# MiloszKrajewski/K4os.Compression.LZ4

Measured on AMD Instinct MI355X. Metric: GiB/s encode+decode on batched 64 KiB blocks; bit-exact vs C# ref, higher is better.
Workload: dtype u8

## Files before the change

### k4os/compression/lz4_amd/csrc/k4lz4_capi.hip

```cpp
#include <hip/hip_runtime.h>
#include <stdint.h>
#include <stdio.h>
#include <stdlib.h>
#include <string.h>
#include <algorithm>
#include <atomic>
#include <memory>
#include <new>
#include <condition_variable>
#include <functional>
#include <mutex>
#include <string>
#include <thread>
#include <chrono>
#include <vector>

#include "../../../../include/k4lz4.h"
#include "k4lz4_decode.hpp"
#include "k4lz4_encode_fast.hpp"
#include "k4lz4_parse.hpp"
#include "k4lz4_pickle.hpp"
#include "k4lz4_segments.hpp"
#include "k4lz4_encode_hc.hpp"
#include "k4lz4_fast_chain.hpp"
// ... 10 lines not shown
#include "k4lz4_selftest.hpp"

constexpr int MAX_PARTS = 8;

struct k4lz4_ctx {
    int device = -1;
    std::string error;
    hipStream_t stream = nullptr;
    int accel = 1;
    unsigned long long *prof = nullptr;
    bool prof_pair = false;
    bool prof_stamp = false;
    uint8_t *d_src = nullptr; size_t d_src_cap = 0;
    uint8_t *d_dst = nullptr; size_t d_dst_cap = 0;
    uint8_t *d_meta = nullptr; size_t d_meta_cap = 0;
    uint8_t *h_stage = nullptr; size_t h_stage_cap = 0;
    uint8_t *d_sched = nullptr; size_t d_sched_cap = 0;
    int cu_count = 256;
    uint8_t *d_dict = nullptr; size_t d_dict_cap = 0;
    uint8_t *d_gtab = nullptr; size_t d_gtab_cap = 0;
    hipStream_t aux = nullptr;
    hipStream_t aux2 = nullptr;
    hipEvent_t ev_join2 = nullptr;
    uint8_t *d_seg = nullptr; size_t d_seg_cap = 0;
    uint8_t *d_seg_first = nullptr; size_t d_seg_first_cap = 0;
    bool use_segments = true;
    uint32_t seg_min = 1024u << 10, seg_target = 640u << 10, seg_warm = 384u << 10;
    uint32_t seg_target_max = 1408u << 10;
    uint32_t seg_spin_max = 0;
    uint32_t seg_div = 3500;
    hipEvent_t ev_fork = nullptr, ev_join = nullptr;
    uint8_t *d_hc_hash = nullptr; size_t d_hc_hash_cap = 0;
    uint8_t *d_hc_work = nullptr; size_t d_hc_work_cap = 0;
    uint8_t *d_hc_meta = nullptr; size_t d_hc_meta_cap = 0;
    uint8_t *d_pk_meta = nullptr; size_t d_pk_meta_cap = 0;
    int pickle_split_min = 512;
    hipEvent_t ev_busy = nullptr;
    hipStream_t last_stream = nullptr;
    bool busy = false;
    uint64_t hc_res_total = 0; uint32_t hc_res_longest = 0;
    uint8_t *h_in[2] = {nullptr, nullptr}; size_t h_in_cap[2] = {0, 0};
    uint8_t *h_out[2] = {nullptr, nullptr}; size_t h_out_cap[2] = {0, 0};
    hipEvent_t ev_in[2] = {nullptr, nullptr}, ev_out[2] = {nullptr, nullptr};
    uint8_t *d_pack = nullptr; size_t d_pack_cap = 0;
    hipStream_t copyq = nullptr;
    hipStream_t dlq = nullptr;
    hipEvent_t ev_up[MAX_PARTS] = {}, ev_len[MAX_PARTS] = {};
    uint8_t *h_len = nullptr; size_t h_len_cap = 0;
    struct Pool *pool = nullptr, *pool_dl = nullptr;
    bool pool_failed = false, pool_dl_failed = false;
    int stage_threads = 7;
    uint32_t *d_pace = nullptr;
    uint32_t *d_status = nullptr;
    int split_pct = -1;
    bool no_pair = false;
    int direct_span_pct = 200;
    bool no_direct = false;
    int lds_floor_per_cu = 8;
    int cost_pct = 48;
    int dec_parts = 4, dec_parts_direct = 8;
    int hop2_max_per_cu = 12;
    bool hc_cand_lds = true;
    int hc_cand_dynlds = 0;
    int hc_segs = 0;
    bool hc_chain_parts = true;
    int hc_mem_pct = 33;
    int pace_min_per_cu = 6;
    bool use_pace = true;
    bool prof_gtab = false;
    uint8_t *d_parse = nullptr; size_t d_parse_cap = 0;
    bool use_parse = true;
    bool parse_queue = false;
    bool hc_records = true;
    bool parse_seg = true;
    bool parse_big = true;
    bool parse_persist = true;
    bool parse_inline_emit = true;
    bool parse_migrate = true;
    bool parse_pcost = false;
    int parse_waves = 16;
    bool trace = false;
    std::vector<uint8_t> h_chain;
    uint8_t *d_chain = nullptr; size_t d_chain_cap = 0;
    hipEvent_t ev_chain = nullptr;
    uint8_t *d_fr = nullptr; size_t d_fr_cap = 0;
    uint8_t *d_fb = nullptr; size_t d_fb_cap = 0;
    uint8_t *d_lg = nullptr; size_t d_lg_cap = 0;
    uint8_t *d_frd = nullptr; size_t d_frd_cap = 0;
    uint8_t *d_lgr = nullptr; size_t d_lgr_cap = 0;
    uint8_t *d_lga = nullptr; size_t d_lga_cap = 0;
    std::vector<uint8_t> h_fw;
    uint8_t *d_fw = nullptr; size_t d_fw_cap = 0;
    hipEvent_t ev_fw = nullptr;
};

struct Pool {
    std::vector<std::thread> workers;
    std::mutex m;
    std::condition_variable cv_work, cv_done;
    std::function<void(int)> job;
    int parts = 0, next = 0, pending = 0;
    unsigned long long gen = 0;
    bool stop = false;
    explicit Pool(int nthreads)
    {
        for (int t = 0; t < nthreads; t++) workers.emplace_back([this] { run(); });
    }
    ~Pool()
    {
        { std::lock_guard<std::mutex> g(m); stop = true; }
        cv_work.notify_all();
        for (auto &w : workers) w.join();
    }
    void run()
    {
        std::unique_lock<std::mutex> lk(m);
        for (;;) {
            cv_work.wait(lk, [this] { return stop || next < parts; });
            if (stop) return;
            const int i = next++;
            lk.unlock();
            job(i);
            lk.lock();
            if (--pending == 0) cv_done.notify_all();
        }
    }
    void parallel(int nparts, const std::function<void(int)> &f)
    {
        if (nparts <= 1 || workers.empty()) { for (int i = 0; i < nparts; i++) f(i); return; }
        std::unique_lock<std::mutex> lk(m);
// ... 344 lines not shown
        if (((kind == KIND_ENCODE && !parse_path) || (K4_DEC_PACE && (kind == KIND_DECODE || kind == KIND_UNPICKLE))) && ctx->use_pace && ctx->d_pace && cnt > (int64_t)ctx->pace_min_per_cu * (int64_t)ctx->cu_count) {
            a.pace = ctx->d_pace;
            K4_HIP(ctx, hipMemsetAsync(a.pace, 0, k4::PACE_BYTES, stream));
        }
        k4::SegArgs sg{};
        bool seg = false;
        if (kind == KIND_ENCODE && (flags & (FLAG_SEGMENTS_OK | K4LZ4_FLAG_SEGMENTS)) && ctx->use_segments && !a.prof && !(flags & K4LZ4_FLAG_ALLOW_COPY)) {
            static_assert(k4::SEG_HDR_DWORDS * 4 == 256, "seg_first_of finds the header in front of the items");
            size_t max_items = (size_t)k4::SEG_MAX_ITEMS;
            if (hostLen) {
                size_t bound = 0;
                for (int64_t i = 0; i < cnt && bound < max_items; i++) {
                    const int32_t u = hostLen[first + i];
                    if (u > 0 && (uint32_t)u >= ctx->seg_min) bound += ((size_t)u + ctx->seg_target - 1) / ctx->seg_target;
                }
                max_items = std::min(max_items, std::max<size_t>(bound, 2));
            }
            const size_t o_items = 256, o_work = o_items + max_items * sizeof(k4::SegItem);
            const size_t o_blocks = o_work + max_items * 4, o_snaps = (o_blocks + (size_t)k4::SEG_MAX_BLOCKS * 4 + 255) & ~(size_t)255;
            const size_t o_tables = o_snaps + max_items * k4::SEG_SNAP_DWORDS * 4, total = o_tables + max_items * 16384;
            if (total > ctx->d_seg_cap || (size_t)cnt * 4 > ctx->d_seg_first_cap) {
                K4_HIP(ctx, hipStreamSynchronize(stream));
                K4_HIP(ctx, hipStreamSynchronize(ctx->aux2));
            }
            int rc = grow(ctx, &ctx->d_seg, &ctx->d_seg_cap, total, false);
            if (rc == K4LZ4_OK) rc = grow(ctx, &ctx->d_seg_first, &ctx->d_seg_first_cap, (size_t)cnt * 4, false);
            if (rc != K4LZ4_OK) return rc;
            sg.hdr = (k4::SegHdr *)ctx->d_seg; sg.items = (k4::SegItem *)(ctx->d_seg + o_items); sg.work = (uint32_t *)(ctx->d_seg + o_work);
            sg.blocks = (uint32_t *)(ctx->d_seg + o_blocks); sg.snaps = (uint32_t *)(ctx->d_seg + o_snaps); sg.tables = (uint32_t *)(ctx->d_seg + o_tables);
            sg.first = (int32_t *)ctx->d_seg_first;
            sg.seg_min = ctx->seg_min; sg.seg_target = ctx->seg_target; sg.seg_warm = ctx->seg_warm; sg.seg_div = ctx->seg_div; sg.seg_target_max = ctx->seg_target_max; sg.spin_max = ctx->seg_spin_max; sg.max_items = (uint32_t)max_items;
            hipLaunchKernelGGL(k4::k4_seg_plan_kernel, dim3(1), dim3(256), 0, stream, a, sg);
            a.seg_first = sg.first; a.seg_items = sg.items; a.seg_snaps = sg.snaps;
            seg = true;
        }
        auto segments_start = [&]() -> int {
            if (!seg) return K4LZ4_OK;
            K4_HIP(ctx, hipEventRecord(ctx->ev_fork, stream));
            K4_HIP(ctx, hipStreamWaitEvent(ctx->aux2, ctx->ev_fork, 0));
            hipLaunchKernelGGL(k4::k4_encode_seg_kernel, dim3((unsigned)((sg.max_items + k4::ENCODE_WAVES_PER_WG - 1) / k4::ENCODE_WAVES_PER_WG)), dim3(64 * k4::ENCODE_WAVES_PER_WG), 0, ctx->aux2, a, sg);
            K4_HIP(ctx, hipEventRecord(ctx->ev_join2, ctx->aux2));
            return K4LZ4_OK;
        };
        auto segments_join = [&]() -> int {
            if (!seg) return K4LZ4_OK;
            K4_HIP(ctx, hipStreamWaitEvent(stream, ctx->ev_join2, 0));
            hipLaunchKernelGGL(k4::k4_seg_join_kernel, dim3((unsigned)std::min<int64_t>(k4::SEG_MAX_BLOCKS, cnt)), dim3(64), 0, stream, a, sg);
            return K4LZ4_OK;
        };
        if (dd && dd->dict) {
            a.dict = dd->dict; a.dictOff = dd->off + first; a.dictLen = dd->len + first;
            a.dictMode = dd->mode ? dd->mode + first : nullptr;
        }
        if (reorder && parse_path && kind == KIND_ENCODE && ctx->parse_pcost) {
            a.cost = d_cost; a.hist = d_hist; a.order_out = d_order;
            K4_HIP(ctx, hipMemsetAsync(d_hist, 0, 2 * k4::PCOST_BUCKETS * 4, stream));
            hipLaunchKernelGGL(k4::k4_pcost_kernel, dim3((unsigned)((cnt + k4::PCOST_WAVES_PER_WG - 1) / k4::PCOST_WAVES_PER_WG)), dim3(64 * k4::PCOST_WAVES_PER_WG), 0, stream, a);
            hipLaunchKernelGGL(k4::k4_porder_kernel, dim3((unsigned)((cnt + 255) / 256)), dim3(256), 0, stream, a);
            a.order = d_order;
        }
        else if (reorder) {
            a.cost = d_cost; a.hist = d_hist; a.order_out = d_order;
            K4_HIP(ctx, hipMemsetAsync(d_hist, 0, (2 * k4::COST_BUCKETS + 16) * 4, stream));
            hipLaunchKernelGGL(k4::k4_cost_kernel, dim3((unsigned)cnt), dim3(64), 0, stream, a, encode_like ? 0 : 1,
                               kind == KIND_ENCODE && parse_path ? k4::COST_SAMPLE_PARSE : k4::COST_SAMPLE);
            const bool two_kernels = kind == KIND_ENCODE && !a.prof && cnt > 512 && !(flags & K4LZ4_FLAG_NO_SPLIT) &&
                                     cnt > 8 * (int64_t)ctx->cu_count && ctx->split_pct <= 0;
            k4::BatchArgs ao = a;
            ao.first = two_kernels ? (uint32_t)ctx->cost_pct : 0u;
            ao.total = (uint32_t)((int64_t)ctx->lds_floor_per_cu * (int64_t)ctx->cu_count);
            hipLaunchKernelGGL(k4::k4_order_kernel, dim3((unsigned)((cnt + 255) / 256)), dim3(256), 0, stream, ao, (uint32_t)lds_share(ctx, cnt));
            a.order = d_order;
            if (two_kernels) a.split = d_hist + 2 * k4::COST_BUCKETS;
        }
        const unsigned wg4 = (unsigned)((cnt + k4::DECODE_WAVES_PER_WG - 1) / k4::DECODE_WAVES_PER_WG);
        bool parse_here = kind == KIND_ENCODE && (parse_path || (parse_seg_path && (a.order || cnt == 1)));
        const bool big_ok = ctx->parse_big && ctx->parse_inline_emit;
        bool any_small = true, any_big = big_ok;
        if (parse_here && hostLen) {
            any_small = false; any_big = false;
            for (int64_t i = 0; i < cnt && !(any_small && (any_big || !big_ok)); i++) {
                const int32_t len = hostLen[first + i];
                if (len >= (int32_t)k4::PARSE_MIN_LEN && len < k4::LIMIT_64K) any_small = true;
                else if (len >= k4::LIMIT_64K && big_ok) any_big = true;
            }
            parse_here = any_small || any_big;
        }
        int64_t waves = 0, nwg = 0, nwg_seg = 0;
        const bool seg_two_step = seg && parse_here && parse_seg_path;
        bool queue = false, slot_recs = false;
        size_t o_meta = 0, o_gtab = 0;
        if (parse_here) {
            waves = std::max<int64_t>(1, std::min<int64_t>(ctx->parse_waves, (cnt + ctx->cu_count - 1) / ctx->cu_count));
            queue = (ctx->parse_queue || parse_persistent || parse_seg_path) && a.order && cnt > waves * (int64_t)ctx->cu_count;
            nwg = queue ? (int64_t)ctx->cu_count : (cnt + waves - 1) / waves;
            if (seg_two_step) nwg_seg = std::min<int64_t>(ctx->cu_count, (cnt + (int64_t)sg.max_items + k4::PARSE_MAX_WAVES - 1) / k4::PARSE_MAX_WAVES);
            slot_recs = ctx->parse_inline_emit;
            const size_t rec_slots = slot_recs ? std::max((size_t)nwg * (size_t)waves, (size_t)nwg_seg * k4::PARSE_MAX_WAVES) : (size_t)cnt;
            o_meta = rec_slots * k4::PARSE_REC_STRIDE * sizeof(uint2); o_gtab = (o_meta + (size_t)cnt * 8 + 64 + 255) & ~(size_t)255;
            const size_t need = o_gtab + std::max(waves > k4::PARSE_LDS_TABLES ? (size_t)nwg * k4::PARSE_MAX_WAVES * 16384 : 0, (size_t)nwg_seg * k4::PARSE_MAX_WAVES * 16384);
            if (need > ctx->d_parse_cap) K4_HIP(ctx, hipStreamSynchronize(stream));
            const int rcp = grow(ctx, &ctx->d_parse, &ctx->d_parse_cap, need, false);
            if (rcp != K4LZ4_OK) { std::lock_guard<std::mutex> g(g_err_mu); ctx->error.clear(); parse_here = false; }
        }
        if (parse_here) {
            k4::ParseArgs pa{};
            pa.recs = (uint2 *)ctx->d_parse; pa.meta = (uint32_t *)(ctx->d_parse + o_meta); pa.gtab = (uint32_t *)(ctx->d_parse + o_gtab);
            pa.nwg = (uint32_t)nwg;
            pa.inline_emit = ctx->parse_inline_emit ? 1u : 0u;
            pa.slot_recs = slot_recs ? 1u : 0u;
            pa.migrate = ctx->parse_migrate ? 1u : 0u;
            pa.big = any_big ? 1u : 0u;
            K4_HIP(ctx, hipMemsetAsync(pa.meta + 2 * cnt, 0, 32, stream));
            if (queue) pa.queue = pa.meta + 2 * cnt;
            pa.nbig = pa.meta + 2 * cnt + 3;
            hipLaunchKernelGGL(k4::k4_parse_kernel, dim3((unsigned)nwg), dim3((unsigned)(64 * waves)), 0, stream, a, pa);
            if (seg_two_step) {
                k4::ParseArgs pb = pa;
                pb.queue = pa.meta + 2 * cnt + 4;
                pb.nwg = (uint32_t)nwg_seg;
                hipLaunchKernelGGL(k4::k4_parse_seg_kernel, dim3((unsigned)nwg_seg), dim3(64 * k4::PARSE_MAX_WAVES), 0, stream, a, pb, sg);
            } else if (any_big) {
                k4::ParseArgs pb = pa;
                if (queue) pb.queue = pa.queue + 4;
                hipLaunchKernelGGL(k4::k4_parse_big_kernel, dim3((unsigned)nwg), dim3((unsigned)(64 * waves)), 0, stream, a, pb);
            }
            if (!pa.inline_emit)
                hipLaunchKernelGGL(k4::k4_emit_kernel, dim3((unsigned)((cnt + k4::EMIT_WAVES_PER_WG - 1) / k4::EMIT_WAVES_PER_WG)), dim3(64 * k4::EMIT_WAVES_PER_WG), 0, stream, a, pa);
            bool rest = true;
            if (hostLen) {
                rest = false;
                for (int64_t i = 0; i < cnt && !rest; i++) rest = hostLen[first + i] < (int32_t)k4::PARSE_MIN_LEN || (hostLen[first + i] >= k4::LIMIT_64K && !any_big);
            }
            if (rest)
                hipLaunchKernelGGL(k4::k4_encode_fast_rest_kernel, dim3((unsigned)((cnt + k4::ENCODE_WAVES_PER_WG - 1) / k4::ENCODE_WAVES_PER_WG)), dim3(64 * k4::ENCODE_WAVES_PER_WG), 0, stream, a, pa);
            if (seg_two_step)
                hipLaunchKernelGGL(k4::k4_seg_join_kernel, dim3((unsigned)std::min<int64_t>(k4::SEG_MAX_BLOCKS, cnt)), dim3(64), 0, stream, a, sg);
            if (flags & K4LZ4_FLAG_ALLOW_COPY)
                hipLaunchKernelGGL(k4::k4_allow_copy_kernel, dim3((unsigned)((cnt + 3) / 4)), dim3(256), 0, stream, a);
            K4_HIP(ctx, hipGetLastError());
            continue;
        }
        switch (kind) {
        case KIND_ENCODE:
            if (a.prof && !ctx->prof_stamp) {
                if (ctx->prof_gtab) {
                    if ((size_t)cnt * 16384 > ctx->d_gtab_cap) {
                        K4_HIP(ctx, hipStreamSynchronize(ctx->aux));
                        int rc2 = grow(ctx, &ctx->d_gtab, &ctx->d_gtab_cap, (size_t)cnt * 16384, false);
                        if (rc2 != K4LZ4_OK) return rc2;
                    }
                    a.gtab = (uint32_t *)ctx->d_gtab;
                }
                hipLaunchKernelGGL(k4::k4_encode_fast_prof_kernel, dim3((unsigned)cnt), dim3(64), 0, stream, a);
            }
            else if (reorder && cnt > 512 && !(flags & K4LZ4_FLAG_NO_SPLIT)) {
                const int64_t lds_slots = 8 * (int64_t)ctx->cu_count;
                const int64_t n_lds = lds_share(ctx, cnt);
                const int64_t n_g = cnt - (a.split ? std::min<int64_t>(cnt, (int64_t)ctx->lds_floor_per_cu * (int64_t)ctx->cu_count) : n_lds);
                const int64_t gchunk = 8192;
                if (n_g > 0 && (size_t)std::min(n_g, gchunk) * 16384 > ctx->d_gtab_cap) {
                    K4_HIP(ctx, hipStreamSynchronize(ctx->aux));
                    int rc2 = grow(ctx, &ctx->d_gtab, &ctx->d_gtab_cap, (size_t)std::min(n_g, gchunk) * 16384, false);
                    if (rc2 != K4LZ4_OK) return rc2;
                }
                { const int rcs = segments_start(); if (rcs != K4LZ4_OK) return rcs; }
// ... 1046 lines not shown
        return rc;
    return s.finish({{outLen, d_out, (size_t)n * 8}}, dst, dstOff, [&](int64_t i) {
        return outLen[i] > 0 && (!capped || (uint64_t)outLen[i] <= dstCap[i]) ? (size_t)outLen[i] : 0;
    });
}

using k4::FW_XXH_BYTES; using k4::FW_CHAIN_LIMIT; using k4::FwAfter;
using k4::fw_ring_at; using k4::fw_slot; using k4::fw_header; using k4::fw_opens; using k4::fw_model; using k4::fw_bound; using k4::fw_code;
using k4::fw_advance;

size_t fw_take(size_t &at, size_t bytes) { const size_t o = at; at += (bytes + 255) & ~(size_t)255; return o; }

}

extern "C" {

int k4lz4_version(void) { return K4LZ4_VERSION; }

void k4lz4_set_enforce32(int on) { g_enforce32.store(on ? 1 : 0, std::memory_order_relaxed); }
int k4lz4_get_enforce32(void) { return g_enforce32.load(std::memory_order_relaxed); }

int k4lz4_device_count(void)
{
    int n = 0;
    if (hipGetDeviceCount(&n) != hipSuccess) { (void)hipGetLastError(); return 0; }
    return n;
}

int k4lz4_ctx_create(k4lz4_ctx **out, int device)
{
    if (!out) return fail(nullptr, K4LZ4_E_ARG, "out is NULL");
    *out = nullptr;
    int n = 0;
    if (hipGetDeviceCount(&n) != hipSuccess || n <= 0) {
        (void)hipGetLastError();
        return fail(nullptr, K4LZ4_E_NO_DEVICE, "no HIP device visible (libk4lz4 has no CPU fallback)");
    }
    if (device < 0) {
        if (hipGetDevice(&device) != hipSuccess) { (void)hipGetLastError(); device = 0; }
    }
    if (device >= n) return fail(nullptr, K4LZ4_E_ARG, "device index out of range");
    hipDeviceProp_t prop;
    K4_HIP(nullptr, hipGetDeviceProperties(&prop, device));
    if (strncmp(prop.gcnArchName, "gfx950", 6) != 0)
        return fail(nullptr, K4LZ4_E_NO_DEVICE, std::string("device is ") + prop.gcnArchName + ", libk4lz4 is built for gfx950 only");
    k4lz4_ctx *ctx = new (std::nothrow) k4lz4_ctx();
    if (!ctx) return fail(nullptr, K4LZ4_E_NOMEM, "out of host memory");
    ctx->device = device;
    ctx->cu_count = prop.multiProcessorCount > 0 ? prop.multiProcessorCount : 256;
    hipError_t e = hipSetDevice(device);
    if (e == hipSuccess) e = hipStreamCreateWithFlags(&ctx->stream, hipStreamNonBlocking);
    if (e == hipSuccess) e = hipMalloc((void **)&ctx->d_status, 64);
    if (e == hipSuccess) e = hipMemset(ctx->d_status, 0, 64);
    if (e == hipSuccess) e = hipMalloc((void **)&ctx->d_pace, k4::PACE_BYTES);
    if (e == hipSuccess) e = hipStreamCreateWithFlags(&ctx->aux, hipStreamNonBlocking);
    if (e == hipSuccess) e = hipStreamCreateWithFlags(&ctx->copyq, hipStreamNonBlocking);
    if (e == hipSuccess) {
        int least = 0, greatest = 0;
        const char *pe = getenv("K4LZ4_SEG_PRIO");
        if ((!pe || atoi(pe) != 0) && hipDeviceGetStreamPriorityRange(&least, &greatest) == hipSuccess && greatest != least)
            e = hipStreamCreateWithPriority(&ctx->aux2, hipStreamNonBlocking, greatest);
        else { (void)hipGetLastError(); e = hipStreamCreateWithFlags(&ctx->aux2, hipStreamNonBlocking); }
    }
    if (e == hipSuccess) e = hipEventCreateWithFlags(&ctx->ev_join2, hipEventDisableTiming);
    if (e == hipSuccess) e = hipEventCreateWithFlags(&ctx->ev_fork, hipEventDisableTiming);
    if (e == hipSuccess) e = hipEventCreateWithFlags(&ctx->ev_join, hipEventDisableTiming);
    if (e == hipSuccess) e = hipEventCreateWithFlags(&ctx->ev_busy, hipEventDisableTiming);
    for (int b = 0; b < 2 && e == hipSuccess; b++) {
        e = hipEventCreateWithFlags(&ctx->ev_in[b], hipEventDisableTiming);
        if (e == hipSuccess) e = hipEventCreateWithFlags(&ctx->ev_out[b], hipEventDisableTiming);
    }
    for (int b = 0; b < MAX_PARTS && e == hipSuccess; b++) {
        e = hipEventCreateWithFlags(&ctx->ev_up[b], hipEventDisableTiming);
        if (e == hipSuccess) e = hipEventCreateWithFlags(&ctx->ev_len[b], hipEventDisableTiming);
    }
    if (e == hipSuccess) e = hipStreamCreateWithFlags(&ctx->dlq, hipStreamNonBlocking);
    if (const char *pct = getenv("K4LZ4_SPLIT_PCT")) { const int v = atoi(pct); ctx->split_pct = v < 1 ? 1 : (v > 100 ? 100 : v); }
    ctx->no_pair = getenv("K4LZ4_NO_PAIR") != nullptr;
    ctx->prof_gtab = getenv("K4LZ4_PROF_GTAB") != nullptr;
    ctx->use_pace = getenv("K4LZ4_NO_PACE") == nullptr;
    if (const char *e = getenv("K4LZ4_PACE_MIN")) ctx->pace_min_per_cu = std::max(0, atoi(e));
    if (const char *e = getenv("K4LZ4_DIRECT_SPAN_PCT")) ctx->direct_span_pct = std::max(100, atoi(e));
    if (const char *e = getenv("K4LZ4_NO_DIRECT")) ctx->no_direct = atoi(e) != 0;
    if (const char *e = getenv("K4LZ4_LDS_FLOOR")) ctx->lds_floor_per_cu = std::max(0, std::min(8, atoi(e)));
    if (const char *e = getenv("K4LZ4_COST_PCT")) ctx->cost_pct = std::max(1, std::min(99, atoi(e)));
    if (const char *e = getenv("K4LZ4_DEC_PARTS")) ctx->dec_parts = std::max(2, std::min(MAX_PARTS, atoi(e)));
    if (const char *e = getenv("K4LZ4_DEC_PARTS_DIRECT")) ctx->dec_parts_direct = std::max(2, std::min(MAX_PARTS, atoi(e)));
    if (const char *e = getenv("K4LZ4_HOP2_MAX")) ctx->hop2_max_per_cu = std::max(0, atoi(e));
    ctx->hc_chain_parts = getenv("K4LZ4_HC_CHAIN_OLD") == nullptr;
    ctx->hc_cand_lds = getenv("K4LZ4_HC_CAND_MEM") == nullptr;
    if (const char *e = getenv("K4LZ4_HC_CAND_DYNLDS")) ctx->hc_cand_dynlds = std::max(0, std::min(65536, atoi(e)));
    if (const char *e = getenv("K4LZ4_HC_SEGS")) { const int v = atoi(e); ctx->hc_segs = v >= 4 ? 4 : (v >= 2 ? 2 : (v == 1 ? 1 : 0)); }
    if (const char *e = getenv("K4LZ4_HC_MEM_PCT")) ctx->hc_mem_pct = std::max(0, std::min(100, atoi(e)));
    ctx->use_segments = getenv("K4LZ4_NO_SEGMENTS") == nullptr;
    if (const char *e = getenv("K4LZ4_SEG_MIN")) ctx->seg_min = (uint32_t)std::max(65536 + 4096, atoi(e));
    if (const char *e = getenv("K4LZ4_SEG_TARGET")) ctx->seg_target = ctx->seg_target_max = (uint32_t)std::max(8192, atoi(e));
    if (const char *e = getenv("K4LZ4_SEG_TARGET_MAX")) ctx->seg_target_max = (uint32_t)std::max(8192, atoi(e));
    if (const char *e = getenv("K4LZ4_SEG_WARM")) ctx->seg_warm = (uint32_t)std::max(0, atoi(e));
    if (const char *e = getenv("K4LZ4_SEG_SPIN_MAX")) ctx->seg_spin_max = (uint32_t)std::max(0, atoi(e));
    if (const char *e = getenv("K4LZ4_SEG_DIV")) ctx->seg_div = (uint32_t)std::max(0, atoi(e));
    if (const char *e = getenv("K4LZ4_PICKLE_SPLIT_MIN")) ctx->pickle_split_min = std::max(0, atoi(e));
    if (const char *e = getenv("K4LZ4_STAGE_THREADS")) ctx->stage_threads = std::max(0, std::min(63, atoi(e) - 1));
    ctx->use_parse = getenv("K4LZ4_NO_PARSE") == nullptr;
    ctx->parse_queue = getenv("K4LZ4_PARSE_QUEUE") != nullptr;
    ctx->parse_persist = getenv("K4LZ4_NO_PERSIST") == nullptr;
    ctx->parse_big = getenv("K4LZ4_NO_PARSE_BIG") == nullptr;
    ctx->parse_seg = getenv("K4LZ4_NO_PARSE_SEG") == nullptr;
    ctx->hc_records = getenv("K4LZ4_NO_HC_RECORDS") == nullptr;
    ctx->parse_pcost = getenv("K4LZ4_PCOST") != nullptr;
    ctx->parse_migrate = getenv("K4LZ4_NO_MIGRATE") == nullptr;
    ctx->parse_inline_emit = getenv("K4LZ4_NO_INLINE_EMIT") == nullptr;
    if (const char *e = getenv("K4LZ4_PARSE_WAVES")) ctx->parse_waves = std::max(1, std::min(k4::PARSE_MAX_WAVES, atoi(e)));
    ctx->trace = getenv("K4LZ4_TRACE") != nullptr;
    if (e != hipSuccess) { delete ctx; return hip_fail(nullptr, e, "hipStreamCreate"); }
    *out = ctx;
    return K4LZ4_OK;
}

void k4lz4_ctx_destroy(k4lz4_ctx *ctx)
{
    if (!ctx) return;
    (void)hipSetDevice(ctx->device);
    if (ctx->stream) { (void)hipStreamSynchronize(ctx->stream); (void)hipStreamDestroy(ctx->stream); }
    if (ctx->aux) { (void)hipStreamSynchronize(ctx->aux); (void)hipStreamDestroy(ctx->aux); }
    if (ctx->aux2) { (void)hipStreamSynchronize(ctx->aux2); (void)hipStreamDestroy(ctx->aux2); }
    if (ctx->ev_join2) (void)hipEventDestroy(ctx->ev_join2);
    if (ctx->d_seg) (void)hipFree(ctx->d_seg);
    if (ctx->d_seg_first) (void)hipFree(ctx->d_seg_first);
    if (ctx->ev_fork) (void)hipEventDestroy(ctx->ev_fork);
    if (ctx->ev_join) (void)hipEventDestroy(ctx->ev_join);
    if (ctx->ev_busy) (void)hipEventDestroy(ctx->ev_busy);
    for (int b = 0; b < 2; b++) {
        if (ctx->ev_in[b]) (void)hipEventDestroy(ctx->ev_in[b]);
        if (ctx->ev_out[b]) (void)hipEventDestroy(ctx->ev_out[b]);
        if (ctx->h_in[b]) (void)hipHostFree(ctx->h_in[b]);
        if (ctx->h_out[b]) (void)hipHostFree(ctx->h_out[b]);
    }
    if (ctx->d_pack) (void)hipFree(ctx->d_pack);
    if (ctx->h_len) (void)hipHostFree(ctx->h_len);
    for (int b = 0; b < MAX_PARTS; b++) {
        if (ctx->ev_up[b]) (void)hipEventDestroy(ctx->ev_up[b]);
        if (ctx->ev_len[b]) (void)hipEventDestroy(ctx->ev_len[b]);
    }
    if (ctx->copyq) (void)hipStreamDestroy(ctx->copyq);
    if (ctx->dlq) (void)hipStreamDestroy(ctx->dlq);
    delete ctx->pool;
    delete ctx->pool_dl;
    if (ctx->d_status) (void)hipFree(ctx->d_status);
    if (ctx->d_pace) (void)hipFree(ctx->d_pace);
    if (ctx->d_gtab) (void)hipFree(ctx->d_gtab);
    if (ctx->d_parse) (void)hipFree(ctx->d_parse);
    if (ctx->d_dict) (void)hipFree(ctx->d_dict);
    if (ctx->d_src) (void)hipFree(ctx->d_src);
    if (ctx->d_dst) (void)hipFree(ctx->d_dst);
    if (ctx->d_meta) (void)hipFree(ctx->d_meta);
    if (ctx->d_fr) (void)hipFree(ctx->d_fr);
    if (ctx->d_fb) (void)hipFree(ctx->d_fb);
    if (ctx->d_lg) (void)hipFree(ctx->d_lg);
    if (ctx->d_frd) (void)hipFree(ctx->d_frd);
    if (ctx->d_lgr) (void)hipFree(ctx->d_lgr);
    if (ctx->d_lga) (void)hipFree(ctx->d_lga);
    if (ctx->h_stage) (void)hipHostFree(ctx->h_stage);
    if (ctx->d_sched) (void)hipFree(ctx->d_sched);
    if (ctx->d_hc_hash) (void)hipFree(ctx->d_hc_hash);
    if (ctx->d_hc_work) (void)hipFree(ctx->d_hc_work);
    if (ctx->d_hc_meta) (void)hipFree(ctx->d_hc_meta);
    if (ctx->d_chain) (void)hipFree(ctx->d_chain);
    if (ctx->d_fw) (void)hipFree(ctx->d_fw);
    if (ctx->ev_fw) (void)hipEventDestroy(ctx->ev_fw);
    if (ctx->ev_chain) (void)hipEventDestroy(ctx->ev_chain);
    if (ctx->d_pk_meta) (void)hipFree(ctx->d_pk_meta);
    delete ctx;
}

const char *k4lz4_last_error(const k4lz4_ctx *ctx) { return ctx ? ctx->error.c_str() : tl_error.c_str(); }

int64_t k4lz4_recommended_min_batch(int kind, int32_t blockBytes, double hostGiBs)
{
    if (kind < 0 || kind > 2 || blockBytes <= 0) return K4LZ4_E_ARG;
    static const double floor_ms_64k[3] = {2.0, 0.55, 2.9};
    static const double box_host_GiBs[3] = {32.0, 35.0, 2.2};
    const double host = hostGiBs > 0.0 ? hostGiBs : box_host_GiBs[kind];
    double floor_ms = floor_ms_64k[kind] * (double)blockBytes / 65536.0;
    if (kind == 0 && blockBytes >= k4::LIMIT_64K) floor_ms = 2.9 * (double)blockBytes / 65536.0;
    if (floor_ms < 0.05) floor_ms = 0.05;
    const double blocks = floor_ms * 1e-3 * host * 1073741824.0 / (double)blockBytes;
    return blocks < 1.0 ? 1 : (int64_t)(blocks + 0.999);
}

int k4lz4_ctx_device(const k4lz4_ctx *ctx) { return ctx ? ctx->device : -1; }

int k4lz4_synchronize(k4lz4_ctx *ctx, void *stream)
{
    if (!ctx) return fail(nullptr, K4LZ4_E_ARG, "ctx is NULL");
    K4_HIP(ctx, hipSetDevice(ctx->device));
    K4_HIP(ctx, hipStreamSynchronize((hipStream_t)stream));
    return take_device_status(ctx);
}

int k4lz4_host_register(void *ptr, size_t bytes)
{
// ... 1815 lines not shown
```

### k4os/compression/lz4_amd/csrc/k4lz4_common.hpp

```cpp
#pragma once
#include <hip/hip_runtime.h>
#include <stdint.h>

namespace k4 {

enum : int {
    MINMATCH = 4,
    LASTLITERALS = 5,
    MFLIMIT = 12,
    MATCH_SAFEGUARD = 12,
    ML_BITS = 4,
    ML_MASK = 15,
    RUN_MASK = 15,
    DISTANCE_MAX = 65535,
    SKIP_TRIGGER = 6,
    LIMIT_64K = 65536 + (MFLIMIT - 1),
    MAX_INPUT_SIZE = 0x7E000000,
};

enum : int {
    FLAG_RAW_RETURN = 1,
    FLAG_PICKLE_WRITER = 2,
    FLAG_X32 = 128,
    FLAG_PARTIAL = 32,
// ... 106 lines not shown

constexpr int PROF_STRIDE = 16;

enum : uint32_t { DEV_STATUS_PIPE_TIMEOUT = 1u, DEV_STATUS_HC_SCRATCH = 2u };
constexpr int HC_NO_SCRATCH = -0x7ffffff1;
__device__ __forceinline__ void dev_status_raise(uint32_t *status, uint32_t bits)
{
    if (status) atomicOr(status, bits);
}

template <bool PROF> __device__ __forceinline__ void prof_place(unsigned long long *pc, int slot, int lane)
{
    if (!PROF || !pc) return;
#ifndef K4_HOST_EMU
    const unsigned long long t = __builtin_amdgcn_s_memrealtime();
    const unsigned hw = __builtin_amdgcn_s_getreg((31 << 11) | 4);
    if (lane == 0) { pc[slot] = t; if (slot == 8) pc[10] = hw; }
#else
    (void)slot; (void)lane;
#endif
}

template <bool PROF> __device__ __forceinline__ unsigned long long prof_now()
{
    if (!PROF) return 0ull;
#if !defined(K4_HOST_EMU) && !defined(K4_PROF_NODRAIN)
    asm volatile("s_waitcnt vmcnt(0) lgkmcnt(0)" ::: "memory");
#endif
    return (unsigned long long)__builtin_readcyclecounter();
}

__device__ __forceinline__ unsigned long long ballot(bool p)
{
#if defined(__HIP_DEVICE_COMPILE__)
    return __builtin_amdgcn_ballot_w64(p);
#else
    return __ballot(p ? 1 : 0);
#endif
}

__device__ __forceinline__ uint32_t uni(uint32_t v) { return __builtin_amdgcn_readfirstlane(v); }
__device__ __forceinline__ uint32_t readlane_u32(uint32_t v, int l) { return (uint32_t)__builtin_amdgcn_readlane(v, l); }
__device__ __forceinline__ int ctz64(unsigned long long m) { return __ffsll(m) - 1; }

__device__ __forceinline__ void agent_publish(uint32_t *p, uint32_t v)
{
#ifndef K4_HOST_EMU
    __threadfence();
    __hip_atomic_store(p, v, __ATOMIC_RELEASE, __HIP_MEMORY_SCOPE_AGENT);
#else
    __atomic_store_n(p, v, __ATOMIC_RELEASE);
#endif
}
__device__ __forceinline__ void agent_acquire()
{
#ifndef K4_HOST_EMU
    __builtin_amdgcn_fence(__ATOMIC_ACQUIRE, "agent");
#else
    __atomic_thread_fence(__ATOMIC_ACQUIRE);
#endif
}
__device__ __forceinline__ uint32_t agent_peek(const uint32_t *p)
{
#ifndef K4_HOST_EMU
    return __hip_atomic_load(p, __ATOMIC_ACQUIRE, __HIP_MEMORY_SCOPE_AGENT);
#else
    return __atomic_load_n(p, __ATOMIC_ACQUIRE);
#endif
}

#ifndef K4_PACE_DEN
#define K4_PACE_DEN 32u
#endif
#ifndef K4_PACE_STEP
#define K4_PACE_STEP 11
#endif
#ifndef K4_PACE_EPOCH
#define K4_PACE_EPOCH 14
#endif
constexpr uint32_t PACE_STEP_LOG2 = K4_PACE_STEP, PACE_EPOCH_LOG2 = K4_PACE_EPOCH;
constexpr uint32_t PACE_SLOTS = 8192, PACE_BYTES = PACE_SLOTS * 16;
struct Pace {
    __device__ __forceinline__ static uint32_t now()
    {
#ifndef K4_HOST_EMU
        return (uint32_t)__builtin_amdgcn_s_memrealtime();
#else
        return 0u;
#endif
    }
    __device__ __forceinline__ static uint32_t *slot_of(uint32_t *base)
    {
#ifndef K4_HOST_EMU
        const uint32_t hw = __builtin_amdgcn_s_getreg((16 << 11) | 4);
        const uint32_t xcc = __builtin_amdgcn_s_getreg((4 << 11) | 20);
        const uint32_t idx = ((hw >> 4) & 3u) | (((hw >> 8) & 0xffu) << 2) | ((xcc & 7u) << 10);
        return base + 4u * idx;
#else
        return base;
#endif
    }
    __device__ __forceinline__ static void begin(uint32_t *base, uint32_t *mine, int lane)
    {
#ifndef K4_HOST_EMU
        if (!base) return;
        const uint32_t t = now();
// ... 258 lines not shown
```

### k4os/compression/lz4_amd/csrc/k4lz4_encode_fast.hpp

```cpp
#pragma once
#include "k4lz4_common.hpp"

namespace k4 {

#ifndef K4_SEG_WAVES_MIN
#define K4_SEG_WAVES_MIN 5
#endif
#ifndef K4_GTAB_DUTY
#define K4_GTAB_DUTY 3
#endif
#ifndef K4_PACE
#define K4_PACE 1
#endif

template <int TYPE> struct FastTable;

template <> struct FastTable<1> {
    uint16_t *t;
    __device__ __forceinline__ static uint32_t hash(const uint8_t *p) { return (ld32u(p) * 2654435761u) >> (32 - 13); }
    __device__ __forceinline__ static uint32_t hash_of(uint32_t seq, uint32_t) { return (seq * 2654435761u) >> (32 - 13); }
    __device__ __forceinline__ uint32_t get(uint32_t h) const { return t[h]; }
    __device__ __forceinline__ void put(uint32_t h, uint32_t pos) const { t[h] = (uint16_t)pos; }
    __device__ __forceinline__ uint32_t get_nt(uint32_t h) const
    {
// ... 770 lines not shown
    if (x32) return encode_fast_block<false, false, true, PAIRS, MORE, N2>(src, src_len, dst, dst_cap, a, ldsw, lane, nullptr, false, nullptr, gtab, pace, sr);
    return encode_fast_block<false, false, false, PAIRS, MORE, N2>(src, src_len, dst, dst_cap, a, ldsw, lane, nullptr, false, nullptr, gtab, pace, sr);
}

__device__ __forceinline__ int codec_encode_result(int src_len, int ret, int flags)
{
    if (flags & FLAG_RAW_RETURN) return ret;
    if (src_len <= 0) return 0;
    return ret <= 0 ? -1 : ret;
}

constexpr int COST_SAMPLE = 512, COST_SAMPLE_PARSE = 256;
constexpr int COST_BUCKETS = 64;

__device__ __forceinline__ uint32_t cost_bucket(unsigned long long cost)
{
    if (cost < 4ull) return (uint32_t)cost;
    const uint32_t l = 63u - (uint32_t)__clzll(cost);
    const uint32_t bkt = 2u * l + (uint32_t)((cost >> (l - 1u)) & 1ull);
    return bkt < (uint32_t)COST_BUCKETS ? bkt : (uint32_t)COST_BUCKETS - 1u;
}

__global__ __launch_bounds__(64) void k4_cost_kernel(BatchArgs a, int by_length, int sample_bytes = COST_SAMPLE)
{
    __shared__ __attribute__((aligned(16))) uint32_t tab[ENCODE_LDS_DWORDS];
    const int lane = lane_id();
    const long long b = (long long)blockIdx.x;
    const int src_len = a.srcLen[b];
    unsigned long long cost = 0;
    if (src_len > 0) {
        if (by_length || src_len <= 64) {
            cost = (unsigned long long)src_len;
        } else {
            const int sample = src_len < sample_bytes ? src_len : sample_bytes;
            uint32_t nseq = 0;
            (void)encode_fast_block<true>(a.src + a.srcOff[b], sample, nullptr, 0x7fffffff, 1u, tab, lane, nullptr, true, &nseq);
            cost = ((unsigned long long)(nseq * 8u + (uint32_t)sample / 16u) * (unsigned long long)src_len) / (unsigned long long)sample;
        }
    }
    if (lane == 0) {
        const uint32_t bkt = cost_bucket(cost);
        a.cost[b] = bkt;
        atomicAdd(&a.hist[bkt], 1u);
    }
}

__device__ __forceinline__ unsigned long long bucket_cost(uint32_t bkt)
{
    if (bkt < 4u) return bkt ? (unsigned long long)bkt * 4ull : 1ull;
    const uint32_t l = bkt >> 1;
    return ((bkt & 1u) ? 7ull : 5ull) << (l - 1u);
}

__global__ __launch_bounds__(256) void k4_order_kernel(BatchArgs a, uint32_t lds_max = 0xffffffffu)
{
    if (blockIdx.x == 0 && threadIdx.x == 0 && a.first != 0u) {
        unsigned long long all = 0;
        for (uint32_t k = 0; k < (uint32_t)COST_BUCKETS; k++) all += (unsigned long long)a.hist[k] * bucket_cost(k);
        const unsigned long long want = all / 100ull * (unsigned long long)a.first;
        unsigned long long have = 0, cnt = 0;
        for (int k = COST_BUCKETS - 1; k >= 0 && have < want; k--) {
            const unsigned long long c = a.hist[k], w = bucket_cost((uint32_t)k);
            if (have + c * w <= want) { have += c * w; cnt += c; }
            else { const unsigned long long part = (want - have + w - 1ull) / w; cnt += part; have = want; }
        }
        const unsigned long long floor_n = (unsigned long long)a.total < (unsigned long long)a.n ? (unsigned long long)a.total : (unsigned long long)a.n;
        if (cnt < floor_n) cnt = floor_n;
        if (cnt > (unsigned long long)a.n) cnt = (unsigned long long)a.n;
        if (cnt > (unsigned long long)lds_max) cnt = (unsigned long long)lds_max;
        a.hist[2 * COST_BUCKETS] = (uint32_t)cnt;
    }
    const long long b = (long long)blockIdx.x * 256 + threadIdx.x;
    if (b >= a.n) return;
    const uint32_t bkt = a.cost[b];
    uint32_t before = 0;
    for (uint32_t k = bkt + 1u; k < (uint32_t)COST_BUCKETS; k++) before += a.hist[k];
    const uint32_t pos = before + atomicAdd(&a.hist[COST_BUCKETS + bkt], 1u);
    a.order_out[pos] = (uint32_t)b;
}

constexpr int ENCODE_WAVES_PER_WG = 2;
struct SegFirst { SegRun run; uint32_t cap; bool cut; };
__device__ __forceinline__ SegFirst seg_first_of(const BatchArgs &a, long long b)
{
    SegFirst f;
    f.cut = false; f.cap = 0u;
    f.run.begin = 0u; f.run.emit_from = 0u; f.run.stop_at = SEG_NONE; f.run.snap_pub = nullptr; f.run.snap_chk = nullptr; f.run.resume = nullptr;
    f.run.cut = 0u; f.run.stop = 0u; f.run.state = 3u; f.run.spin_max = 0u; f.run.fix = nullptr;
    if (!a.seg_first) return f;
    const int32_t it = (int32_t)uni((uint32_t)a.seg_first[b]);
    if (it < 0) return f;
    const uint32_t *w = (const uint32_t *)a.seg_items + SEG_ITEM_WORDS * (uint32_t)it;
    f.cut = true;
    f.run.spin_max = uni(((const uint32_t *)a.seg_items)[-(int)SEG_HDR_DWORDS + 3]);
    f.run.stop_at = uni(w[4]);
    f.cap = f.run.stop_at;
    f.run.snap_chk = a.seg_snaps + (size_t)(it + 1) * SEG_SNAP_DWORDS;
    f.run.fix = a.seg_snaps + (size_t)uni(((const uint32_t *)a.seg_items)[-(int)SEG_HDR_DWORDS + 7]) * SEG_SNAP_DWORDS + 4096ull * (unsigned long long)it;
    return f;
}
__device__ __forceinline__ void seg_first_done(const BatchArgs &a, long long b, const SegFirst &f, int ret, int lane)
{
    if (!f.cut || lane != 0) return;
    uint32_t *w = (uint32_t *)a.seg_items + SEG_ITEM_WORDS * (uint32_t)a.seg_first[b];
    w[6] = f.run.cut; w[7] = f.run.stop; w[8] = ret > 0 ? f.run.state : 3u; w[9] = (uint32_t)ret;
}

template <bool MORE, bool SEG = false>
__device__ __forceinline__ void encode_fast_kernel_body(const BatchArgs &a, uint32_t (*tabs)[ENCODE_LDS_DWORDS])
{
    const int lane = lane_id();
    const uint32_t wave = uni(threadIdx.x >> 6);
    const long long slot = (long long)blockIdx.x * ENCODE_WAVES_PER_WG + (long long)wave;
    if (slot >= a.n || (a.split && slot >= (long long)uni(*a.split))) return;
    uint32_t *tab = tabs[wave];
    const long long b = a.order ? (long long)uni(a.order[slot]) : slot;
    const int src_len = a.srcLen[b];
    const int cap = a.dstCap[b];
    const uint8_t *src = a.src + a.srcOff[b];
    uint8_t *dst = a.dst + a.dstOff[b];
    int ret = 0;
    if (a.prof) { prof_place<true>(a.prof + PROF_STRIDE * b, 8, lane); if (lane == 0) a.prof[PROF_STRIDE * b + 11] = MORE ? 3u : 1u; }
    if (SEG) {
        SegFirst f = seg_first_of(a, b);
        const int c = cap < 0 ? 0 : (f.cut && (uint32_t)cap > f.cap ? (int)f.cap : cap);
        if (src_len > 0 || (a.flags & FLAG_RAW_RETURN))
            ret = compress_fast_block<true, MORE>(src, src_len, dst, c, a.accel, tab, lane, nullptr, (a.flags & FLAG_X32) != 0, a.pace, &f.run);
        seg_first_done(a, b, f, ret, lane);
    } else
    if (src_len > 0 || (a.flags & FLAG_RAW_RETURN))
        ret = compress_fast_block<true, MORE>(src, src_len, dst, cap < 0 ? 0 : cap, a.accel, tab, lane, nullptr, (a.flags & FLAG_X32) != 0, a.pace);
// ... 77 lines not shown
```

Measured before the change: 60.96.

## Fuse cost, order and meta zeroing into one last-block prelude kernel

For encode batches on the parse path that fit within the parse wave capacity, the memset, cost kernel, order kernel and meta memset are replaced by a single prelude kernel. Each wave samples one block's cost and adds to a persistent device histogram, and the last workgroup to finish (found with an atomic ticket) scans the buckets, computes the split count, scatters the order and resets the state. This removes several launches and the host-side memset from the critical path. In exchange, the ordering is done by one workgroup, cross-block visibility depends on release/acquire fences, and the order within a bucket comes from LDS atomics.

Measured after the change: 61.16 (median of 6 runs). About the same (+0.3%).

```diff
diff --git a/k4os/compression/lz4_amd/csrc/k4lz4_capi.hip b/k4os/compression/lz4_amd/csrc/k4lz4_capi.hip
--- a/k4os/compression/lz4_amd/csrc/k4lz4_capi.hip
+++ b/k4os/compression/lz4_amd/csrc/k4lz4_capi.hip
@@ -86,6 +86,7 @@
     int stage_threads = 7;
     uint32_t *d_pace = nullptr;
     uint32_t *d_status = nullptr;
+    uint32_t *d_prelude = nullptr;
     int split_pct = -1;
     bool no_pair = false;
     int direct_span_pct = 200;
@@ -110,6 +111,7 @@
     bool parse_big = true;
     bool parse_persist = true;
     bool parse_inline_emit = true;
+    bool parse_prelude = true;
     bool parse_migrate = true;
     bool parse_pcost = false;
     int parse_waves = 16;
@@ -560,6 +562,15 @@
             a.dict = dd->dict; a.dictOff = dd->off + first; a.dictLen = dd->len + first;
             a.dictMode = dd->mode ? dd->mode + first : nullptr;
         }
+        bool prelude_pending = false;
+        k4::BatchArgs ao{};
+        auto cost_and_order = [&]() -> int {
+            K4_HIP(ctx, hipMemsetAsync(d_hist, 0, (2 * k4::COST_BUCKETS + 16) * 4, stream));
+            hipLaunchKernelGGL(k4::k4_cost_kernel, dim3((unsigned)cnt), dim3(64), 0, stream, ao, encode_like ? 0 : 1,
+                               kind == KIND_ENCODE && parse_path ? k4::COST_SAMPLE_PARSE : k4::COST_SAMPLE);
+            hipLaunchKernelGGL(k4::k4_order_kernel, dim3((unsigned)((cnt + 255) / 256)), dim3(256), 0, stream, ao, (uint32_t)lds_share(ctx, cnt));
+            return K4LZ4_OK;
+        };
         if (reorder && parse_path && kind == KIND_ENCODE && ctx->parse_pcost) {
             a.cost = d_cost; a.hist = d_hist; a.order_out = d_order;
             K4_HIP(ctx, hipMemsetAsync(d_hist, 0, 2 * k4::PCOST_BUCKETS * 4, stream));
@@ -569,15 +580,13 @@
         }
         else if (reorder) {
             a.cost = d_cost; a.hist = d_hist; a.order_out = d_order;
-            K4_HIP(ctx, hipMemsetAsync(d_hist, 0, (2 * k4::COST_BUCKETS + 16) * 4, stream));
-            hipLaunchKernelGGL(k4::k4_cost_kernel, dim3((unsigned)cnt), dim3(64), 0, stream, a, encode_like ? 0 : 1,
-                               kind == KIND_ENCODE && parse_path ? k4::COST_SAMPLE_PARSE : k4::COST_SAMPLE);
             const bool two_kernels = kind == KIND_ENCODE && !a.prof && cnt > 512 && !(flags & K4LZ4_FLAG_NO_SPLIT) &&
                                      cnt > 8 * (int64_t)ctx->cu_count && ctx->split_pct <= 0;
-            k4::BatchArgs ao = a;
+            ao = a;
             ao.first = two_kernels ? (uint32_t)ctx->cost_pct : 0u;
             ao.total = (uint32_t)((int64_t)ctx->lds_floor_per_cu * (int64_t)ctx->cu_count);
-            hipLaunchKernelGGL(k4::k4_order_kernel, dim3((unsigned)((cnt + 255) / 256)), dim3(256), 0, stream, ao, (uint32_t)lds_share(ctx, cnt));
+            prelude_pending = kind == KIND_ENCODE && parse_path && !seg && ctx->parse_prelude && cnt <= (int64_t)k4::PARSE_MAX_WAVES * (int64_t)ctx->cu_count;
+            if (!prelude_pending) { const int rco = cost_and_order(); if (rco != K4LZ4_OK) return rco; }
             a.order = d_order;
             if (two_kernels) a.split = d_hist + 2 * k4::COST_BUCKETS;
         }
@@ -611,6 +620,11 @@
             const int rcp = grow(ctx, &ctx->d_parse, &ctx->d_parse_cap, need, false);
             if (rcp != K4LZ4_OK) { std::lock_guard<std::mutex> g(g_err_mu); ctx->error.clear(); parse_here = false; }
         }
+        if (prelude_pending && !parse_here) {
+            prelude_pending = false;
+            const int rco = cost_and_order();
+            if (rco != K4LZ4_OK) return rco;
+        }
         if (parse_here) {
             k4::ParseArgs pa{};
             pa.recs = (uint2 *)ctx->d_parse; pa.meta = (uint32_t *)(ctx->d_parse + o_meta); pa.gtab = (uint32_t *)(ctx->d_parse + o_gtab);
@@ -619,7 +633,10 @@
             pa.slot_recs = slot_recs ? 1u : 0u;
             pa.migrate = ctx->parse_migrate ? 1u : 0u;
             pa.big = any_big ? 1u : 0u;
-            K4_HIP(ctx, hipMemsetAsync(pa.meta + 2 * cnt, 0, 32, stream));
+            if (prelude_pending)
+                hipLaunchKernelGGL(k4::k4_prelude_kernel, dim3((unsigned)((cnt + k4::PRELUDE_WAVES - 1) / k4::PRELUDE_WAVES)), dim3(64 * k4::PRELUDE_WAVES), 0, stream,
+                                   ao, (uint32_t)lds_share(ctx, cnt), ctx->d_prelude, pa.meta + 2 * cnt);
+            else K4_HIP(ctx, hipMemsetAsync(pa.meta + 2 * cnt, 0, 32, stream));
             if (queue) pa.queue = pa.meta + 2 * cnt;
             pa.nbig = pa.meta + 2 * cnt + 3;
             hipLaunchKernelGGL(k4::k4_parse_kernel, dim3((unsigned)nwg), dim3((unsigned)(64 * waves)), 0, stream, a, pa);
@@ -1772,6 +1789,8 @@
     if (e == hipSuccess) e = hipStreamCreateWithFlags(&ctx->stream, hipStreamNonBlocking);
     if (e == hipSuccess) e = hipMalloc((void **)&ctx->d_status, 64);
     if (e == hipSuccess) e = hipMemset(ctx->d_status, 0, 64);
+    if (e == hipSuccess) e = hipMalloc((void **)&ctx->d_prelude, k4::PRELUDE_STATE_WORDS * 4);
+    if (e == hipSuccess) e = hipMemset(ctx->d_prelude, 0, k4::PRELUDE_STATE_WORDS * 4);
     if (e == hipSuccess) e = hipMalloc((void **)&ctx->d_pace, k4::PACE_BYTES);
     if (e == hipSuccess) e = hipStreamCreateWithFlags(&ctx->aux, hipStreamNonBlocking);
     if (e == hipSuccess) e = hipStreamCreateWithFlags(&ctx->copyq, hipStreamNonBlocking);
@@ -1829,6 +1848,7 @@
     ctx->hc_records = getenv("K4LZ4_NO_HC_RECORDS") == nullptr;
     ctx->parse_pcost = getenv("K4LZ4_PCOST") != nullptr;
     ctx->parse_migrate = getenv("K4LZ4_NO_MIGRATE") == nullptr;
+    ctx->parse_prelude = getenv("K4LZ4_NO_PRELUDE") == nullptr;
     ctx->parse_inline_emit = getenv("K4LZ4_NO_INLINE_EMIT") == nullptr;
     if (const char *e = getenv("K4LZ4_PARSE_WAVES")) ctx->parse_waves = std::max(1, std::min(k4::PARSE_MAX_WAVES, atoi(e)));
     ctx->trace = getenv("K4LZ4_TRACE") != nullptr;
@@ -1867,6 +1887,7 @@
     delete ctx->pool;
     delete ctx->pool_dl;
     if (ctx->d_status) (void)hipFree(ctx->d_status);
+    if (ctx->d_prelude) (void)hipFree(ctx->d_prelude);
     if (ctx->d_pace) (void)hipFree(ctx->d_pace);
     if (ctx->d_gtab) (void)hipFree(ctx->d_gtab);
     if (ctx->d_parse) (void)hipFree(ctx->d_parse);
diff --git a/k4os/compression/lz4_amd/csrc/k4lz4_common.hpp b/k4os/compression/lz4_amd/csrc/k4lz4_common.hpp
--- a/k4os/compression/lz4_amd/csrc/k4lz4_common.hpp
+++ b/k4os/compression/lz4_amd/csrc/k4lz4_common.hpp
@@ -182,6 +182,14 @@
     __atomic_store_n(p, v, __ATOMIC_RELEASE);
 #endif
 }
+__device__ __forceinline__ void agent_release()
+{
+#ifndef K4_HOST_EMU
+    __builtin_amdgcn_fence(__ATOMIC_RELEASE, "agent");
+#else
+    __atomic_thread_fence(__ATOMIC_RELEASE);
+#endif
+}
 __device__ __forceinline__ void agent_acquire()
 {
 #ifndef K4_HOST_EMU
diff --git a/k4os/compression/lz4_amd/csrc/k4lz4_encode_fast.hpp b/k4os/compression/lz4_amd/csrc/k4lz4_encode_fast.hpp
--- a/k4os/compression/lz4_amd/csrc/k4lz4_encode_fast.hpp
+++ b/k4os/compression/lz4_amd/csrc/k4lz4_encode_fast.hpp
@@ -846,24 +846,27 @@
     return ((bkt & 1u) ? 7ull : 5ull) << (l - 1u);
 }
 
+__device__ __forceinline__ uint32_t cost_split(const uint32_t *hist, uint32_t pct, uint32_t floor_total, long long n, uint32_t lds_max)
+{
+    unsigned long long all = 0;
+    for (uint32_t k = 0; k < (uint32_t)COST_BUCKETS; k++) all += (unsigned long long)hist[k] * bucket_cost(k);
+    const unsigned long long want = all / 100ull * (unsigned long long)pct;
+    unsigned long long have = 0, cnt = 0;
+    for (int k = COST_BUCKETS - 1; k >= 0 && have < want; k--) {
+        const unsigned long long c = hist[k], w = bucket_cost((uint32_t)k);
+        if (have + c * w <= want) { have += c * w; cnt += c; }
+        else { const unsigned long long part = (want - have + w - 1ull) / w; cnt += part; have = want; }
+    }
+    const unsigned long long floor_n = (unsigned long long)floor_total < (unsigned long long)n ? (unsigned long long)floor_total : (unsigned long long)n;
+    if (cnt < floor_n) cnt = floor_n;
+    if (cnt > (unsigned long long)n) cnt = (unsigned long long)n;
+    if (cnt > (unsigned long long)lds_max) cnt = (unsigned long long)lds_max;
+    return (uint32_t)cnt;
+}
+
 __global__ __launch_bounds__(256) void k4_order_kernel(BatchArgs a, uint32_t lds_max = 0xffffffffu)
 {
-    if (blockIdx.x == 0 && threadIdx.x == 0 && a.first != 0u) {
-        unsigned long long all = 0;
-        for (uint32_t k = 0; k < (uint32_t)COST_BUCKETS; k++) all += (unsigned long long)a.hist[k] * bucket_cost(k);
-        const unsigned long long want = all / 100ull * (unsigned long long)a.first;
-        unsigned long long have = 0, cnt = 0;
-        for (int k = COST_BUCKETS - 1; k >= 0 && have < want; k--) {
-            const unsigned long long c = a.hist[k], w = bucket_cost((uint32_t)k);
-            if (have + c * w <= want) { have += c * w; cnt += c; }
-            else { const unsigned long long part = (want - have + w - 1ull) / w; cnt += part; have = want; }
-        }
-        const unsigned long long floor_n = (unsigned long long)a.total < (unsigned long long)a.n ? (unsigned long long)a.total : (unsigned long long)a.n;
-        if (cnt < floor_n) cnt = floor_n;
-        if (cnt > (unsigned long long)a.n) cnt = (unsigned long long)a.n;
-        if (cnt > (unsigned long long)lds_max) cnt = (unsigned long long)lds_max;
-        a.hist[2 * COST_BUCKETS] = (uint32_t)cnt;
-    }
+    if (blockIdx.x == 0 && threadIdx.x == 0 && a.first != 0u) a.hist[2 * COST_BUCKETS] = cost_split(a.hist, a.first, a.total, a.n, lds_max);
     const long long b = (long long)blockIdx.x * 256 + threadIdx.x;
     if (b >= a.n) return;
     const uint32_t bkt = a.cost[b];
@@ -871,6 +874,60 @@
     for (uint32_t k = bkt + 1u; k < (uint32_t)COST_BUCKETS; k++) before += a.hist[k];
     const uint32_t pos = before + atomicAdd(&a.hist[COST_BUCKETS + bkt], 1u);
     a.order_out[pos] = (uint32_t)b;
+}
+
+constexpr int PRELUDE_WAVES = 8;
+constexpr int PRELUDE_STATE_WORDS = COST_BUCKETS + 1;
+__global__ __launch_bounds__(64 * PRELUDE_WAVES) void k4_prelude_kernel(BatchArgs a, uint32_t lds_max, uint32_t *state, uint32_t *zero8)
+{
+    __shared__ __attribute__((aligned(16))) uint32_t tabs[PRELUDE_WAVES][ENCODE_LDS_DWORDS];
+    __shared__ uint32_t last;
+    const int lane = lane_id();
+    const uint32_t wave = uni(threadIdx.x >> 6);
+    const long long b = (long long)blockIdx.x * PRELUDE_WAVES + (long long)wave;
+    if (b < a.n) {
+        const int src_len = a.srcLen[b];
+        unsigned long long cost = 0;
+        if (src_len > 64) {
+            const int sample = src_len < COST_SAMPLE_PARSE ? src_len : COST_SAMPLE_PARSE;
+            uint32_t nseq = 0;
+            (void)encode_fast_block<true>(a.src + a.srcOff[b], sample, nullptr, 0x7fffffff, 1u, tabs[wave], lane, nullptr, true, &nseq);
+            cost = ((unsigned long long)(nseq * 8u + (uint32_t)sample / 16u) * (unsigned long long)src_len) / (unsigned long long)sample;
+        } else if (src_len > 0) {
+            cost = (unsigned long long)src_len;
+        }
+        if (lane == 0) {
+            const uint32_t bkt = cost_bucket(cost);
+            a.cost[b] = bkt;
+            atomicAdd(&state[bkt], 1u);
+        }
+    }
+    agent_release();
+    __syncthreads();
+    if (threadIdx.x == 0) {
+        last = atomicAdd(&state[COST_BUCKETS], 1u) == gridDim.x - 1u ? 1u : 0u;
+    }
+    __syncthreads();
+    if (!last) return;
+    agent_acquire();
+    uint32_t *hist = tabs[0], *before = hist + COST_BUCKETS, *cursor = before + COST_BUCKETS;
+    if (wave == 0) {
+        const uint32_t k = (uint32_t)(COST_BUCKETS - 1 - lane);
+        const uint32_t c = agent_peek(&state[k]);
+        state[k] = 0u;
+        hist[k] = c; cursor[k] = 0u;
+        before[k] = wave_inclusive_scan(c) - c;
+        if (lane == 0) state[COST_BUCKETS] = 0u;
+        if (lane < 8 && zero8) zero8[lane] = 0u;
+    }
+    static_assert(COST_BUCKETS == 64 && PRELUDE_WAVES >= 2, "one lane per bucket; the split by a second wave");
+    __syncthreads();
+    if (threadIdx.x == 64u && a.first != 0u)
+        a.hist[2 * COST_BUCKETS] = cost_split(hist, a.first, a.total, a.n, lds_max);
+    for (long long i = (long long)threadIdx.x; i < a.n; i += 64 * PRELUDE_WAVES) {
+        const uint32_t bkt = agent_peek(&a.cost[i]);
+        a.order_out[before[bkt] + atomicAdd(&cursor[bkt], 1u)] = (uint32_t)i;
+    }
 }
 
 constexpr int ENCODE_WAVES_PER_WG = 2;
```
